# intel-aero/aero-optical-flow

Measured on AMD Instinct MI355X. Metric: frame-pairs/s (640x480, 8x8 SAD, +-4 search), higher is better.
Workload: dtype u8

## Files before the change

aero-optical-flow_amd/csrc/k_reduce.hip:

```cpp
#include "aof_device.hpp"
#include "aof_internal.hpp"
#include "aof_reduce.hpp"

namespace aof {

namespace {

constexpr int kThreads = 256;
constexpr int kMaxHist = 256;
constexpr int64_t kMidPairs = 1024;
constexpr int64_t kWidePairs = 512;

template <int GROUP, int kThreads = 256>
__global__ __launch_bounds__(kThreads) void k_reduce(ReduceArgs a)
{
    constexpr int kGroups = kThreads / GROUP;
    __shared__ uint32_t s_hist[kGroups][2][kMaxHist];
    __shared__ int s_sums[kGroups][3];
    const int grp = (int)threadIdx.x / GROUP, tid = (int)threadIdx.x % GROUP;
    const int64_t pair = (int64_t)blockIdx.x * kGroups + grp;
    if (GROUP < kThreads && pair >= a.n_pairs) return;
    auto sync = [] { if (GROUP == kThreads) __syncthreads(); else __builtin_amdgcn_wave_barrier(); };
    uint32_t (*hist)[kMaxHist] = s_hist[grp];
    int *sums = s_sums[grp];
    const int centre = 2 * a.tail.range + 1, n = 2 * centre + 1;
    for (int k = tid; k < n; k += GROUP) { hist[0][k] = 0; hist[1][k] = 0; }
    if (tid < 3) sums[tid] = 0;
    sync();

    if (a.parts) {
        const uint32_t *parts = a.parts + (size_t)pair * a.nstrips * (size_t)(2 * n);
        for (int k = tid; k < 2 * n; k += GROUP) {
            uint32_t v = 0;
            for (int st = 0; st < a.nstrips; st++) v += parts[(size_t)st * (2 * n) + k];
            const int axis = k >= n, bin = k - axis * n;
            hist[axis][bin] = v;
            if (v) {
                atomicAdd(&sums[axis], (bin - centre) * (int)v);
                if (!axis) atomicAdd(&sums[2], (int)v);
            }
        }
        sync();
    } else {
    const aof_block *blocks = a.blocks + pair * a.tail.nblocks;
    const uint8_t *subdirs = a.subdirs ? a.subdirs + pair * a.tail.nblocks : nullptr;
    int s2x = 0, s2y = 0, cnt = 0;
    auto vote = [&](bool ok, aof_block r, int sd) {
        ok = ok && !(r.sad == AOF_SAD_SKIPPED || (int)r.sad >= a.value_threshold);
        int hx = 0, hy = 0;
        if (ok && subdirs) {
            hx = (sd == 0 || sd == 1 || sd == 7) ? 1 : ((sd == 3 || sd == 4 || sd == 5) ? -1 : 0);
            hy = (sd == 1 || sd == 2 || sd == 3) ? 1 : ((sd == 5 || sd == 6 || sd == 7) ? -1 : 0);
        }
        const int vx = 2 * r.dx + hx, vy = 2 * r.dy + hy;
        wave_vote2(hist[0], hist[1], vx + centre, vy + centre, ok);
        if (ok) { s2x += vx; s2y += vy; cnt++; }
    };
    typedef uint32_t u32_bytes __attribute__((aligned(1)));
    const uint32_t *words = reinterpret_cast<const uint32_t *>(blocks);
    const int quads = a.tail.nblocks / 4;
    const int qrounds = (quads + GROUP - 1) / GROUP;
    auto vote_quad = [&](bool have, const uint32_t (&w)[4], uint32_t sd4) {
        int key[4], weight = 0, first = 0;
        bool ok[4], messy = false;
#pragma unroll
        for (int j = 0; j < 4; j++) {
            const uint32_t sad = w[j] >> 16;
            ok[j] = have && !(sad == AOF_SAD_SKIPPED || (int)sad >= a.value_threshold);
            const int sd = (int)((sd4 >> (8 * j)) & 0xFFu);
            int hx = 0, hy = 0;
            if (subdirs) {
                hx = (sd == 0 || sd == 1 || sd == 7) ? 1 : ((sd == 3 || sd == 4 || sd == 5) ? -1 : 0);
                hy = (sd == 1 || sd == 2 || sd == 3) ? 1 : ((sd == 5 || sd == 6 || sd == 7) ? -1 : 0);
            }
            const int vx = 2 * (int)(int8_t)(w[j] & 0xFFu) + hx, vy = 2 * (int)(int8_t)((w[j] >> 8) & 0xFFu) + hy;
            key[j] = (vx + centre) | ((vy + centre) << 16);
            if (ok[j]) {
                s2x += vx; s2y += vy; cnt++;
                if (weight == 0) first = key[j];
                else if (key[j] != first) messy = true;
                weight++;
            }
        }
        if (__ballot(messy) == 0) {
            wave_vote2_weighted(hist[0], hist[1], first, weight);
        } else {
#pragma unroll
            for (int j = 0; j < 4; j++) wave_vote2(hist[0], hist[1], key[j] & 0xFFFF, key[j] >> 16, ok[j]);
        }
    };
    constexpr int kBatchQ = 3;
    for (int it0 = 0; it0 < qrounds; it0 += kBatchQ) {
        uint32_t rec[kBatchQ][4], sdir[kBatchQ];
#pragma unroll
        for (int k = 0; k < kBatchQ; k++) {
            const int q = (it0 + k) * GROUP + tid;
#pragma unroll
            for (int j = 0; j < 4; j++) rec[k][j] = 0xFFFF0000u;
            sdir[k] = 0x08080808u;
            if (it0 + k < qrounds && q < quads) {
                __builtin_memcpy(rec[k], words + 4 * q, 16);
                if (subdirs) sdir[k] = *reinterpret_cast<const u32_bytes *>(subdirs + 4 * q);
            }
        }
#pragma unroll
        for (int k = 0; k < kBatchQ; k++) {
            if (it0 + k >= qrounds) break;
            const int q = (it0 + k) * GROUP + tid;
            vote_quad(q < quads, rec[k], sdir[k]);
        }
    }
    {
        const int b = 4 * quads + tid;
        const bool in = b < a.tail.nblocks;
        aof_block r;
        r.dx = 0; r.dy = 0; r.sad = AOF_SAD_SKIPPED;
        if (in) r = blocks[b];
        vote(in, r, in && subdirs ? subdirs[b] : 8);
    }
    s2x = (int)wave_sum_u32((uint32_t)s2x);
    s2y = (int)wave_sum_u32((uint32_t)s2y);
    cnt = (int)wave_sum_u32((uint32_t)cnt);
    if ((tid & 63) == 0) {
        atomicAdd(&sums[0], s2x);
        atomicAdd(&sums[1], s2y);
        atomicAdd(&sums[2], cnt);
    }
    sync();
    }
    if (n <= 64) {
        if (tid < 64) finalise_flow_wave(a.tail, pair, hist[0], hist[1], sums);
    } else if (tid == 0) {
        finalise_flow(a.tail, pair, hist[0], hist[1], sums);
    }
}

__global__ __launch_bounds__(kThreads) void k_reduce_chunk(ReduceArgs a, int chunks)
{
    __shared__ uint32_t hist[2][kMaxHist];
    const int chunk = (int)(blockIdx.x % (uint32_t)chunks);
    const int64_t pair = (int64_t)(blockIdx.x / (uint32_t)chunks);
    const int tid = threadIdx.x;
    const int centre = 2 * a.tail.range + 1, n = 2 * centre + 1;
    for (int k = tid; k < n; k += kThreads) { hist[0][k] = 0; hist[1][k] = 0; }
    __syncthreads();
    const int per = (a.tail.nblocks + chunks - 1) / chunks;
    const int b0 = chunk * per, b1 = min(a.tail.nblocks, b0 + per);
    const uint32_t *blocks = reinterpret_cast<const uint32_t *>(a.blocks) + pair * a.tail.nblocks;
    const uint8_t *subdirs = a.subdirs ? a.subdirs + pair * a.tail.nblocks : nullptr;
    for (int base = b0; base < b1; base += kThreads) {
        const int b = base + tid;
        const bool in = b < b1;
        const aof_block r = __builtin_bit_cast(aof_block, in ? blocks[b] : 0xFFFF0000u);
        const int sd = in && subdirs ? subdirs[b] : 8;
        const bool ok = in && !(r.sad == AOF_SAD_SKIPPED || (int)r.sad >= a.value_threshold);
        int hx = 0, hy = 0;
        if (ok && subdirs) {
            hx = (sd == 0 || sd == 1 || sd == 7) ? 1 : ((sd == 3 || sd == 4 || sd == 5) ? -1 : 0);
            hy = (sd == 1 || sd == 2 || sd == 3) ? 1 : ((sd == 5 || sd == 6 || sd == 7) ? -1 : 0);
        }
        wave_vote(hist[0], 2 * r.dx + hx + centre, ok);
        wave_vote(hist[1], 2 * r.dy + hy + centre, ok);
    }
    __syncthreads();
    uint32_t *out = a.chunk_parts + ((size_t)pair * chunks + chunk) * (size_t)(2 * n);
    for (int k = tid; k < 2 * n; k += kThreads) out[k] = k < n ? hist[0][k] : hist[1][k - n];
}

}

int launch_reduce(const ReduceArgs &a, void *stream)
{
    if (a.n_pairs == 0) return 0;
    if (a.n_pairs > 0x7FFFFFFF) return (int)hipErrorInvalidValue;
    const int chunks = a.parts ? 0 : reduce_chunks(a.tail.nblocks);
    if (chunks > 0 && a.chunk_parts && a.n_pairs * chunks <= 0x7FFFFFFF) {
        hipLaunchKernelGGL(k_reduce_chunk, dim3((uint32_t)(a.n_pairs * chunks)), dim3(kThreads), 0,
                           static_cast<hipStream_t>(stream), a, chunks);
        ReduceArgs b = a;
        b.parts = a.chunk_parts;
        b.nstrips = chunks;
        hipLaunchKernelGGL(k_reduce<kThreads>, dim3((uint32_t)a.n_pairs), dim3(kThreads), 0,
                           static_cast<hipStream_t>(stream), b);
        return (int)hipGetLastError();
    }
    if (a.tail.nblocks <= 256 && !a.parts)
        hipLaunchKernelGGL(k_reduce<64>, dim3((uint32_t)((a.n_pairs + 3) / 4)), dim3(kThreads), 0,
                           static_cast<hipStream_t>(stream), a);
    else if (a.n_pairs <= kWidePairs && a.tail.nblocks >= 2048 && !a.parts)
        hipLaunchKernelGGL((k_reduce<1024, 1024>), dim3((uint32_t)a.n_pairs), dim3(1024), 0,
                           static_cast<hipStream_t>(stream), a);
    else if (a.n_pairs <= kMidPairs && a.tail.nblocks >= 2048 && !a.parts)
        hipLaunchKernelGGL((k_reduce<512, 512>), dim3((uint32_t)a.n_pairs), dim3(512), 0,
                           static_cast<hipStream_t>(stream), a);
    else
        hipLaunchKernelGGL(k_reduce<kThreads>, dim3((uint32_t)a.n_pairs), dim3(kThreads), 0,
                           static_cast<hipStream_t>(stream), a);
    return (int)hipGetLastError();
}

}
```

Baseline: 7.977 million.

## Add register-packed bitfield histogram reduce kernel replacing LDS atomic voting

Adds a new reduce kernel that accumulates per-lane vote histograms as packed 3-bit and 6-bit fields inside 64-bit registers instead of LDS atomics. The packed counts are then reduced across the wave with DPP and permlane swaps and combined across waves through a small shared array before finalisation. The goal is to remove the shared-memory atomic contention and ballot overhead of the per-vote histogram. It applies only when the bin count and block count fit the field widths, and it depends on the threshold word comparison and the bit packing staying exact.

```diff
diff --git a/aero-optical-flow_amd/csrc/aof_reduce_fields.hpp b/aero-optical-flow_amd/csrc/aof_reduce_fields.hpp
--- /dev/null
+++ b/aero-optical-flow_amd/csrc/aof_reduce_fields.hpp
@@ -0,0 +1,45 @@
+#pragma once
+
+#include "aof_hd.hpp"
+
+namespace aof {
+
+constexpr int kFieldsMaxBins = 19;
+constexpr int kFieldsMaxBlocks = 8192;
+constexpr int kFieldsMinBlocks = 257;
+constexpr int kFieldsMinLanes = 256;
+constexpr int kFieldsQuadBits = 3, kFieldsLaneBits = 6, kFieldsWaveBits = 16;
+constexpr int kFieldsWave = 64;
+
+AOF_HD_INLINE constexpr int reduce_lanes(long long n_pairs, int nblocks)
+{
+    return nblocks >= 2048 && n_pairs <= 512 ? 1024 : nblocks >= 2048 && n_pairs <= 1024 ? 512 : 256;
+}
+
+AOF_HD_INLINE constexpr int fields_quad_rounds(int nblocks, int lanes) { return (nblocks / 4 + lanes - 1) / lanes; }
+
+AOF_HD_INLINE constexpr int fields_quad_records(int nblocks) { return 4 + (nblocks % 4 ? 1 : 0); }
+
+AOF_HD_INLINE constexpr int fields_lane_records(int nblocks, int lanes)
+{
+    return 4 * fields_quad_rounds(nblocks, lanes) + (nblocks % 4 ? 1 : 0);
+}
+
+AOF_HD_INLINE constexpr int fields_max(int bits) { return (1 << bits) - 1; }
+
+AOF_HD_INLINE constexpr bool fields_fit(int nblocks, int lanes, int bins)
+{
+    return nblocks >= kFieldsMinBlocks && nblocks <= kFieldsMaxBlocks && lanes >= kFieldsMinLanes && bins <= kFieldsMaxBins &&
+           bins * kFieldsQuadBits <= 64 && ((bins + 1) / 2) * kFieldsLaneBits <= 64 &&
+           fields_quad_rounds(nblocks, lanes) * lanes <= kFieldsMaxBlocks / 4 &&
+           fields_quad_records(nblocks) <= fields_max(kFieldsQuadBits) &&
+           fields_lane_records(nblocks, lanes) <= fields_max(kFieldsLaneBits) &&
+           kFieldsWave * fields_lane_records(nblocks, lanes) <= fields_max(kFieldsWaveBits);
+}
+
+static_assert(fields_lane_records(kFieldsMaxBlocks, kFieldsMinLanes) == 32 && fields_lane_records(kFieldsMaxBlocks - 1, kFieldsMinLanes) == 33, "");
+static_assert(fields_fit(kFieldsMaxBlocks, kFieldsMinLanes, kFieldsMaxBins) && fields_fit(kFieldsMaxBlocks - 1, kFieldsMinLanes, kFieldsMaxBins), "");
+static_assert(fields_fit(kFieldsMinBlocks, 256, kFieldsMaxBins) && fields_fit(2048, 1024, kFieldsMaxBins) && fields_fit(kFieldsMaxBlocks, 512, kFieldsMaxBins), "");
+static_assert(!fields_fit(kFieldsMaxBlocks + 1, 256, kFieldsMaxBins) && !fields_fit(256, 256, kFieldsMaxBins) && !fields_fit(4661, 512, kFieldsMaxBins + 2), "");
+
+}
diff --git a/aero-optical-flow_amd/csrc/k_reduce.hip b/aero-optical-flow_amd/csrc/k_reduce.hip
--- a/aero-optical-flow_amd/csrc/k_reduce.hip
+++ b/aero-optical-flow_amd/csrc/k_reduce.hip
@@ -1,6 +1,7 @@
 #include "aof_device.hpp"
 #include "aof_internal.hpp"
 #include "aof_reduce.hpp"
+#include "aof_reduce_fields.hpp"
 
 namespace aof {
 
@@ -8,8 +9,6 @@
 
 constexpr int kThreads = 256;
 constexpr int kMaxHist = 256;
-constexpr int64_t kMidPairs = 1024;
-constexpr int64_t kWidePairs = 512;
 
 template <int GROUP, int kThreads = 256>
 __global__ __launch_bounds__(kThreads) void k_reduce(ReduceArgs a)
@@ -133,6 +132,144 @@
     } else if (tid == 0) {
         finalise_flow(a.tail, pair, hist[0], hist[1], sums);
     }
+}
+
+
+__device__ __forceinline__ void fields_vote(uint32_t w, uint32_t thr_word, int shift3_x, int shift3_y, uint64_t &qx, uint64_t &qy)
+{
+    const uint64_t ok = w < thr_word ? 1u : 0u;
+    qx += ok << ((6u * (w & 31u) + (uint32_t)shift3_x) & 63u);
+    qy += ok << ((6u * ((w >> 8) & 31u) + (uint32_t)shift3_y) & 63u);
+}
+
+constexpr uint32_t fields_half_table(bool y)
+{
+    uint32_t t = 0;
+    for (int sd = 0; sd <= 8; sd++) {
+        const int hx = (sd == 0 || sd == 1 || sd == 7) ? 1 : ((sd == 3 || sd == 4 || sd == 5) ? -1 : 0);
+        const int hy = (sd == 1 || sd == 2 || sd == 3) ? 1 : ((sd == 5 || sd == 6 || sd == 7) ? -1 : 0);
+        t |= (uint32_t)((y ? hy : hx) + 1) << (2 * sd);
+    }
+    return t;
+}
+constexpr uint32_t kHalfTableX = fields_half_table(false), kHalfTableY = fields_half_table(true);
+static_assert(kHalfTableX == 0x1901Au && kHalfTableY == 0x101A9u, "");
+__device__ __forceinline__ int fields_half3_x(uint32_t sd) { return 3 * (int)((kHalfTableX >> (2 * (sd > 8u ? 8u : sd))) & 3u); }
+__device__ __forceinline__ int fields_half3_y(uint32_t sd) { return 3 * (int)((kHalfTableY >> (2 * (sd > 8u ? 8u : sd))) & 3u); }
+
+template <int HALF, int DPP>
+__device__ __forceinline__ void fields_halve(const uint32_t (&v)[2 * HALF], uint32_t (&out)[HALF], bool upper)
+{
+#pragma unroll
+    for (int i = 0; i < HALF; i++) {
+        const uint32_t lo = v[i] + (uint32_t)__builtin_amdgcn_update_dpp(0, (int)v[i], DPP, 0xF, 0xF, false);
+        const uint32_t hi = v[i + HALF] + (uint32_t)__builtin_amdgcn_update_dpp(0, (int)v[i + HALF], DPP, 0xF, 0xF, false);
+        out[i] = upper ? hi : lo;
+    }
+}
+constexpr int kDppXor8 = 0x128, kDppXor7 = 0x141, kDppXor2 = 0x4E, kDppXor1 = 0xB1;
+
+__device__ __forceinline__ uint32_t fields_wave_sum(uint32_t v)
+{
+    v += (uint32_t)__builtin_amdgcn_update_dpp(0, (int)v, kDppXor1, 0xF, 0xF, false);
+    v += (uint32_t)__builtin_amdgcn_update_dpp(0, (int)v, kDppXor2, 0xF, 0xF, false);
+    v += (uint32_t)__builtin_amdgcn_update_dpp(0, (int)v, kDppXor7, 0xF, 0xF, false);
+    v += (uint32_t)__builtin_amdgcn_update_dpp(0, (int)v, kDppXor8, 0xF, 0xF, false);
+    const auto rows = __builtin_amdgcn_permlane16_swap(v, v, false, false);
+    v = rows[0] + rows[1];
+    const auto halves = __builtin_amdgcn_permlane32_swap(v, v, false, false);
+    return halves[0] + halves[1];
+}
+
+template <int LANES, bool HALFPEL>
+__global__ __launch_bounds__(LANES) void k_reduce_fields(ReduceArgs a)
+{
+    constexpr int kWaves = LANES / kFieldsWave;
+    constexpr int kRounds = kFieldsMaxBlocks / 4 / LANES;
+    static_assert(fields_fit(kFieldsMaxBlocks, LANES, kFieldsMaxBins) && fields_quad_rounds(kFieldsMaxBlocks, LANES) == kRounds, "");
+    __shared__ uint32_t s_totals[kWaves][kFieldsWave];
+    const int tid = (int)threadIdx.x, lane = tid & 63;
+    const int64_t pair = blockIdx.x;
+    const int nblocks = a.tail.nblocks, quads = nblocks / 4;
+    const int centre = 2 * a.tail.range + 1;
+    const uint32_t *words = reinterpret_cast<const uint32_t *>(a.blocks + pair * nblocks);
+    const uint8_t *subdirs = HALFPEL ? a.subdirs + pair * nblocks : nullptr;
+    typedef uint32_t u32_bytes __attribute__((aligned(1)));
+
+    uint32_t rec[kRounds][4], sdir[kRounds], tail_rec = 0xFFFF0000u, tail_sd = 8;
+#pragma unroll
+    for (int k = 0; k < kRounds; k++) {
+        const int q = k * LANES + tid;
+#pragma unroll
+        for (int j = 0; j < 4; j++) rec[k][j] = 0xFFFF0000u;
+        sdir[k] = 0x08080808u;
+        if (q < quads) {
+            __builtin_memcpy(rec[k], words + 4 * q, 16);
+            if (HALFPEL) sdir[k] = *reinterpret_cast<const u32_bytes *>(subdirs + 4 * q);
+        }
+    }
+    if (4 * quads + tid < nblocks) {
+        tail_rec = words[4 * quads + tid];
+        if (HALFPEL) tail_sd = subdirs[4 * quads + tid];
+    }
+
+    const int vt = a.value_threshold;
+    const uint32_t thr_word = (uint32_t)(vt < 0 ? 0 : (vt > 0xFFFF ? 0xFFFF : vt)) << 16;
+    const int c3 = 3 * centre - (HALFPEL ? 3 : 0);
+    uint64_t ex = 0, ox = 0, ey = 0, oy = 0;
+    constexpr uint64_t kEven = 0x71C71C71C71C71C7ull;
+#pragma unroll
+    for (int k = 0; k < kRounds; k++) {
+        if (k * LANES >= quads) break;
+        uint64_t qx = 0, qy = 0;
+#pragma unroll
+        for (int j = 0; j < 4; j++) {
+            const uint32_t sd = (sdir[k] >> (8 * j)) & 0xFFu;
+            fields_vote(rec[k][j], thr_word, c3 + (HALFPEL ? fields_half3_x(sd) : 0), c3 + (HALFPEL ? fields_half3_y(sd) : 0), qx, qy);
+        }
+        if (k == 0)
+            fields_vote(tail_rec, thr_word, c3 + (HALFPEL ? fields_half3_x(tail_sd) : 0), c3 + (HALFPEL ? fields_half3_y(tail_sd) : 0), qx, qy);
+        ex += qx & kEven; ox += (qx >> 3) & kEven;
+        ey += qy & kEven; oy += (qy >> 3) & kEven;
+    }
+
+    uint32_t vx[16], vy[16];
+#pragma unroll
+    for (int d = 0; d < 16; d++) {
+        vx[d] = d < 10 ? (uint32_t)((ex >> (6 * d)) & 63u) | ((uint32_t)((ox >> (6 * d)) & 63u) << 16) : 0u;
+        vy[d] = d < 10 ? (uint32_t)((ey >> (6 * d)) & 63u) | ((uint32_t)((oy >> (6 * d)) & 63u) << 16) : 0u;
+    }
+    uint32_t v16[16], v8[8], v4[4], v2[2], v1[1];
+#pragma unroll
+    for (int d = 0; d < 16; d++) {
+        v16[d] = 0;
+        if (d < 10) {
+            const auto r = __builtin_amdgcn_permlane32_swap(vx[d], vy[d], false, false);
+            v16[d] = r[0] + r[1];
+        }
+    }
+#pragma unroll
+    for (int i = 0; i < 8; i++) {
+        const auto r = __builtin_amdgcn_permlane16_swap(v16[i], v16[i + 8], false, false);
+        v8[i] = r[0] + r[1];
+    }
+    fields_halve<4, kDppXor8>(v8, v4, (lane & 8) != 0);
+    fields_halve<2, kDppXor7>(v4, v2, (lane & 4) != 0);
+    fields_halve<1, kDppXor2>(v2, v1, (lane & 2) != 0);
+    const uint32_t both = v1[0] + (uint32_t)__builtin_amdgcn_update_dpp(0, (int)v1[0], kDppXor1, 0xF, 0xF, false);
+    const uint32_t mine = (lane & 1) ? both >> 16 : both & 0xFFFFu;
+    s_totals[tid >> 6][lane] = mine;
+    __syncthreads();
+    if (tid >= kFieldsWave) return;
+    uint32_t total = 0;
+#pragma unroll
+    for (int w = 0; w < kWaves; w++) total += s_totals[w][lane];
+    const uint32_t other = (uint32_t)__shfl((int)total, lane ^ 32, 64);
+    const uint32_t hx = lane < 32 ? total : 0u, hy = lane < 32 ? other : 0u;
+    const int count = (int)fields_wave_sum(hx);
+    const int sum2x = (int)fields_wave_sum((uint32_t)((lane - centre) * (int)hx));
+    const int sum2y = (int)fields_wave_sum((uint32_t)((lane - centre) * (int)hy));
+    finalise_flow_wave_bins(a.tail, pair, hx, hy, sum2x, sum2y, count);
 }
 
 __global__ __launch_bounds__(kThreads) void k_reduce_chunk(ReduceArgs a, int chunks)
@@ -184,18 +321,33 @@
                            static_cast<hipStream_t>(stream), b);
         return (int)hipGetLastError();
     }
-    if (a.tail.nblocks <= 256 && !a.parts)
+    if (a.tail.nblocks <= 256 && !a.parts) {
         hipLaunchKernelGGL(k_reduce<64>, dim3((uint32_t)((a.n_pairs + 3) / 4)), dim3(kThreads), 0,
                            static_cast<hipStream_t>(stream), a);
-    else if (a.n_pairs <= kWidePairs && a.tail.nblocks >= 2048 && !a.parts)
-        hipLaunchKernelGGL((k_reduce<1024, 1024>), dim3((uint32_t)a.n_pairs), dim3(1024), 0,
-                           static_cast<hipStream_t>(stream), a);
-    else if (a.n_pairs <= kMidPairs && a.tail.nblocks >= 2048 && !a.parts)
-        hipLaunchKernelGGL((k_reduce<512, 512>), dim3((uint32_t)a.n_pairs), dim3(512), 0,
-                           static_cast<hipStream_t>(stream), a);
-    else
-        hipLaunchKernelGGL(k_reduce<kThreads>, dim3((uint32_t)a.n_pairs), dim3(kThreads), 0,
-                           static_cast<hipStream_t>(stream), a);
+        return (int)hipGetLastError();
+    }
+    const int lanes = a.parts ? kThreads : reduce_lanes(a.n_pairs, a.tail.nblocks);
+    const dim3 grid((uint32_t)a.n_pairs);
+    hipStream_t s = static_cast<hipStream_t>(stream);
+    if (!a.parts && fields_fit(a.tail.nblocks, lanes, 2 * (2 * a.tail.range + 1) + 1)) {
+        const bool half = a.subdirs != nullptr;
+        if (lanes == 1024) {
+            if (half) hipLaunchKernelGGL((k_reduce_fields<1024, true>), grid, dim3(1024), 0, s, a);
+            else hipLaunchKernelGGL((k_reduce_fields<1024, false>), grid, dim3(1024), 0, s, a);
+        } else if (lanes == 512) {
+            if (half) hipLaunchKernelGGL((k_reduce_fields<512, true>), grid, dim3(512), 0, s, a);
+            else hipLaunchKernelGGL((k_reduce_fields<512, false>), grid, dim3(512), 0, s, a);
+        } else {
+            if (half) hipLaunchKernelGGL((k_reduce_fields<256, true>), grid, dim3(256), 0, s, a);
+            else hipLaunchKernelGGL((k_reduce_fields<256, false>), grid, dim3(256), 0, s, a);
+        }
+    } else if (lanes == 1024) {
+        hipLaunchKernelGGL((k_reduce<1024, 1024>), grid, dim3(1024), 0, s, a);
+    } else if (lanes == 512) {
+        hipLaunchKernelGGL((k_reduce<512, 512>), grid, dim3(512), 0, s, a);
+    } else {
+        hipLaunchKernelGGL(k_reduce<kThreads>, grid, dim3(kThreads), 0, s, a);
+    }
     return (int)hipGetLastError();
 }
 
```

Result: faster. 8.077 million, median of 6 (+1.3%).
